# Algolzw/image-restoration-sde

Hardware: AMD Instinct MI355X
Metric: restored images/sec at 256x256, 100-step IR-SDE reverse sampler (higher is better)
Workload: dtype f32; 1 GPU; IR-SDE deraining ConditionalUNet nf=64 depth=4, reverse_sde, batch=16/GPU 256x256, T=100 (BASELINE.json configs[1]); compute_dtype=fp32, global_batch=16

## Files before the change

### image_restoration_sde_amd/csrc/common.h

```cpp
#pragma once
#include <hip/hip_runtime.h>
#include <cstdint>
#include <cstdio>
#include <cstdlib>
#include <stdexcept>
#include <string>
#include <vector>
#include "split3_layout.h"

namespace irsde {

struct HipError : std::runtime_error {
    using std::runtime_error::runtime_error;
};
struct HipOutOfMemory : HipError {
    using HipError::HipError;
};

inline int tuning_env_int(const char* name, int dflt) {
    static const bool on = [] { const char* t = getenv("IRSDE_TUNING"); return t && atoi(t) == 1; }();
    if (!on) return dflt;
    const char* v = getenv(name);
    return v ? atoi(v) : dflt;
}
// ... 77 lines not shown
struct WinoPolyParams {
    int up = 0;
    const float* in = nullptr;
    int C = 0, Hin = 0, Win = 0;
    int B = 0, TH = 0, TW = 0, T = 0;
    float* V = nullptr;
    unsigned short* Vs = nullptr;
    int thread_writer = 0;
    const float* M = nullptr;
    int Cout = 0, Ho = 0, Wo = 0;
    float* out = nullptr;
    int out_stride = 0;
    const float* bias = nullptr;
};
void launch_wino_poly_input(const WinoPolyParams& p, hipStream_t s);
void launch_wino_poly_output(const WinoPolyParams& p, hipStream_t s);
void wino_poly_transform_weights(const float* w_packed, int Cout, int Cin, float* U, int up);
struct SplitGemmArgs {
    const unsigned short* a = nullptr;
    const unsigned short* b = nullptr;
    float* out = nullptr;
    long long plA = 0, plB = 0, pA = 0, pB = 0, pO = 0;
    int M = 0, N = 0, K = 0, lda = 0, ldc = 0;
    float out_scale = 1.f;
    int n_inner = 1;
    int nblk_n = 0;
};
void gemm_split_global_init();
int gemm_split_inner(int M, int N, int ncomp);
void launch_gemm_split_pairs(const SplitGemmArgs& a, int ncomp, hipStream_t s, int abl = 0, bool f16 = false);
void launch_split_pairs(const float* in, unsigned short* out, size_t rows, int K, hipStream_t s, bool f16 = false,
                        float scale = 1.0f);
void launch_gemm_split(const SplitGemmArgs& a, int nplanes, int ncomp, hipStream_t s);
void launch_gemm_split_triples(const SplitGemmArgs& a, int ncomp, hipStream_t s, int abl = 0, int walk = -1);
void set_force_split3_blocks(int n);
bool gemm_split_triples_fits(long long M, long long N, long long K, long long ldc);
void launch_split_triples(const float* in, unsigned short* out, int ncomp, size_t rows, int K, hipStream_t s);
void launch_split_planes(const float* in, unsigned short* out, size_t n, size_t plane, int nplanes, hipStream_t s, bool f16 = false,
                         float scale = 1.0f);
void launch_wino_output(const WinoParams& p, hipStream_t s);
void wino_transform_weights(const float* w_packed, int Cout, int Cin, float* U, int tile);
bool wino_fused_eligible(const ConvParams& p);
void wino_fused_pack_weights(const float* U, int Cout, int Cin, float* Uf);
void launch_wino_fused(const ConvParams& p, const float* Uf, hipStream_t s, unsigned long long* dbg = nullptr, int dflags = 0);
int wino_fused_num_blocks(const ConvParams& p);
bool wino_fused64_eligible(const ConvParams& p);
void wino_fused64_pack_weights(const float* U, int Cout, int Cin, float* Uf);
void launch_wino_fused64(const ConvParams& p, const float* Uf, hipStream_t s, int variant = 0);
void wino_fused64_set_debug(unsigned long long* buf);
constexpr float kWinoFused64PairVScale = 0.0625f;
void launch_wino_fused64_split_weights(const float* Uf, unsigned short* out, size_t nfloats, float scale, hipStream_t s);
int wino_fused64_num_blocks(const ConvParams& p);
bool wino_fused64_xcd_nb(const ConvParams& p);
void wino_fused_global_init();
int device_cu_count();
bool wino_fused64t_eligible(const ConvParams& p);
long long wino_fused64t_num_items(const ConvParams& p);
void launch_wino_fused64t(const ConvParams& p, const float* Uf, hipStream_t s, int variant = 0);
void wino_fused64t_set_debug(unsigned long long* buf);
void wino_fused_t_global_init();
void naf_chain_global_init();
void naf_chain_set_debug(unsigned long long* buf);
bool naf_chain_shape_ok(int H, int W, int c);
size_t naf_chain_weight_halves(int nblocks);
size_t naf_chain_vec_floats(int nblocks);
void launch_naf_chain(const float* x, float* out, const unsigned short* w, const float* vecs, int nblocks, int B, const float* film, int film_bstride,
                      int film_off, const float* cam, int cam_bstride, int cam_off, hipStream_t s, int variant = 0);
// ... 156 lines not shown
```

### image_restoration_sde_amd/csrc/engine_debug.hip

```cpp
#include "engine.h"
#include "../../include/irsde_hip_debug.h"

using namespace irsde;

namespace irsde {
namespace {

struct Scratch {
    hipStream_t s;
    std::vector<void*> bufs;
    explicit Scratch(hipStream_t s_) : s(s_) {}
    ~Scratch() {
        (void)hipStreamSynchronize(s);
        for (void* p : bufs) (void)hipFree(p);
    }
    Scratch(const Scratch&) = delete;
    Scratch& operator=(const Scratch&) = delete;
    template <class T> T* alloc(size_t n) {
        void* p = nullptr;
        IRSDE_HIP_CHECK(hipMalloc(&p, n * sizeof(T)));
        bufs.push_back(p);
        return static_cast<T*>(p);
    }
    float* upload(const float* host, size_t n) {
// ... 20 lines not shown
        if (e0) (void)hipEventDestroy(e0);
        if (e1) (void)hipEventDestroy(e1);
    }
    EventPair(const EventPair&) = delete;
    EventPair& operator=(const EventPair&) = delete;
};
template <class Run>
double time_launches(hipStream_t s, int iters, Run&& run) {
    EventPair ev;
    IRSDE_HIP_CHECK(hipEventRecord(ev.e0, s));
    for (int i = 0; i < iters; ++i) run();
    IRSDE_HIP_CHECK(hipEventRecord(ev.e1, s));
    IRSDE_HIP_CHECK(hipStreamSynchronize(s));
    float ms = 0.f;
    IRSDE_HIP_CHECK(hipEventElapsedTime(&ms, ev.e0, ev.e1));
    return ms / iters;
}

struct VariantScope {
    explicit VariantScope(int v) { conv_set_variant(v); }
    ~VariantScope() { conv_set_variant(0); }
};

bool code_in(const std::initializer_list<int>& codes, int c) { return std::find(codes.begin(), codes.end(), c) != codes.end(); }
bool debug_conv_code_known(int c) {
    return code_in({0, 1, 2, 3, 4, 5, 12, 13, 22, 23, 24, 25, 26, 27, 28, 48, 33, 34, 35, 36, 37, 42, 43, 44, 45, 46, 47, 55, 56, 62, 63, 204, 260, 261, 262, 263}, c) ||
           code_in({100, 103, 105, 106, 107, 150, 160, 161, 162, 163, 165, 166, 167, 170, 171, 172, 173}, c);
}
bool bench_conv_variant_known(int v) {
    return code_in({0, 3, 5, 6, 7, 50, 60, 61, 62, 63, 64, 65, 66, 67, 70, 71, 72, 73}, v) ||
           code_in({80, 81, 82, 412, 413, 421, 422, 423, 430, 431, 432, 434, 435, 460, 461, 462, 465, 467, 468, 469, 480, 481, 482}, v) ||
           code_in({2001, 2002, 2004, 4650, 4651, 4652, 4653}, v) ||
           (v >= 83 && v <= 82 + 255) ||
           (v >= 490 && v <= 499) ||
           (v >= 472 && v <= 476);
}

struct ScamHookArgs {
    const float* x;
    float* out;
    const float *norm_l_g, *norm_r_g, *l_proj1_w, *l_proj1_b, *r_proj1_w, *r_proj1_b, *l_proj2_w, *l_proj2_b, *r_proj2_w, *r_proj2_b, *beta, *gamma;
};
struct ScamHookDev {
    float *gl, *gr, *beta, *gamma;
    float *in2, *qv, *F;
    size_t vsz;
};
template <class ShapeCheck, class Prologue, class Tail>
void scam_hook(const ScamHookArgs& a, int B, int Hs, int Ws, int C, void* stream, ShapeCheck check_shape, Prologue prologue, Tail tail) {
    if (!a.x || !a.out || !a.norm_l_g || !a.norm_r_g || !a.l_proj1_w || !a.l_proj1_b || !a.r_proj1_w || !a.r_proj1_b || !a.l_proj2_w || !a.l_proj2_b ||
        !a.r_proj2_w || !a.r_proj2_b || !a.beta || !a.gamma)
        throw HipError("null argument");
    check_shape();
    hipStream_t s = reinterpret_cast<hipStream_t>(stream);
    conv_global_init();
    std::vector<float> wl, bl, wr, br;
    scam_pack_proj(a.l_proj1_w, a.l_proj1_b, a.l_proj2_w, a.l_proj2_b, C, wl, bl);
    scam_pack_proj(a.r_proj1_w, a.r_proj1_b, a.r_proj2_w, a.r_proj2_b, C, wr, br);
    Scratch mem(s);
    auto up = [&](const float* h, size_t n) {
        float* d = mem.alloc<float>(std::max<size_t>(n, 16));
        if (h) IRSDE_HIP_CHECK(hipMemcpy(d, h, n * 4, hipMemcpyHostToDevice));
        return d;
    };
    ScamHookDev d;
    d.gl = up(a.norm_l_g, C); d.gr = up(a.norm_r_g, C); d.beta = up(a.beta, C); d.gamma = up(a.gamma, C);
    float *dwl = up(wl.data(), wl.size()), *dbl = up(bl.data(), bl.size()), *dwr = up(wr.data(), wr.size()), *dbr = up(br.data(), br.size());
// ... 434 lines not shown
            if (f16) {
                unsigned short* dbf = mem.alloc<unsigned short>(pk.size());
                launch_f32_to_f16(dw, dbf, pk.size(), s);
                p.w_bf = dbf;
                p.f16 = 1;
            }
            const size_t npix_in = (size_t)B * Hin * Win, nout = (size_t)B * p.Ho * p.Wo * Cout;
            if (act) {
                auto to_bf = [&](const float* src, size_t n) {
                    unsigned short* d = mem.alloc<unsigned short>(n + 32);
                    launch_f32_to_bf16(src, d, n, s);
                    return reinterpret_cast<const float*>(d);
                };
                p.in0 = to_bf(in0, npix_in * C0);
                if (in1) p.in1 = to_bf(in1, npix_in * C1);
                if (res) p.res = to_bf(res, nout);
                ao = mem.alloc<unsigned short>(nout + 32);
                p.out = reinterpret_cast<float*>(ao);
                p.in_bf16 = p.out_bf16 = 1;
            }
            {
                const int halo_v = (naive == 162 || naive == 262 || naive == 166) ? 64 : (naive == 163 || naive == 263 || naive == 167) ? 65 : 0;
                VariantScope vs(halo_v ? halo_v : f16 ? (naive == 165 ? 61 : 0) : act ? (naive == 204 ? 0 : naive - 200) : (naive >= 100 ? naive - 100 : 0));
                launch_conv(p, s);
            }
            if (act) launch_bf16_to_f32(ao, out, nout, s);
        }
        IRSDE_HIP_CHECK(hipStreamSynchronize(s));
    });
}

int irsde_debug_split_gemm(const float* A, const float* Bm, float* C, int M, int N, int K, int ncomp, int nplanes, void* stream) {
    return guard([&] {
        if (nplanes != 2 && nplanes != 3 && (nplanes < 42 || nplanes > 45)) throw HipError("debug_split_gemm: nplanes must be 2, 3, 42, 43, 44 or 45");
        hipStream_t s = reinterpret_cast<hipStream_t>(stream);
        conv_global_init();
        const size_t na = (size_t)ncomp * M * K, nb = (size_t)ncomp * N * K;
        Scratch mem(s);
        if (nplanes == 43 || nplanes == 45) {
            if (!gemm_split_triples_fits(M, N, K, N)) throw HipError("debug_split_gemm: shape not eligible for the three-piece GEMM");
            const size_t ea = split3_comp_elems((size_t)M, (size_t)K), eb = split3_comp_elems((size_t)N, (size_t)K);
            unsigned short *ta = mem.alloc<unsigned short>(ea * ncomp), *tb = mem.alloc<unsigned short>(eb * ncomp);
            launch_split_triples(A, ta, ncomp, (size_t)M, K, s);
            launch_split_triples(Bm, tb, ncomp, (size_t)N, K, s);
            SplitGemmArgs gt;
            gt.a = ta; gt.b = tb; gt.out = C;
            gt.pA = (long long)ea; gt.pB = (long long)eb; gt.pO = (long long)M * N;
            gt.M = M; gt.N = N; gt.K = K; gt.lda = K; gt.ldc = N;
            launch_gemm_split_triples(gt, ncomp, s, 0, nplanes == 45 ? 0 : -1);
            IRSDE_HIP_CHECK(hipStreamSynchronize(s));
            return;
        }
        if (nplanes == 42 || nplanes == 44) {
            const bool f16 = nplanes == 44;
            const float sa = f16 ? 1.0f / 16.0f : 1.f, sb = f16 ? 64.0f : 1.f;
            unsigned short *pa = mem.alloc<unsigned short>(2 * na), *pb = mem.alloc<unsigned short>(2 * nb);
            launch_split_pairs(A, pa, (size_t)ncomp * M, K, s, f16, sa);
            launch_split_pairs(Bm, pb, (size_t)ncomp * N, K, s, f16, sb);
            SplitGemmArgs gp;
            gp.a = pa; gp.b = pb; gp.out = C;
            gp.pA = (long long)M * K; gp.pB = (long long)N * K; gp.pO = (long long)M * N;
            gp.M = M; gp.N = N; gp.K = K; gp.lda = K; gp.ldc = N;
            gp.out_scale = 1.0f / (sa * sb);
            launch_gemm_split_pairs(gp, ncomp, s, 0, f16);
            IRSDE_HIP_CHECK(hipStreamSynchronize(s));
            return;
        }
        unsigned short *da = mem.alloc<unsigned short>(na * nplanes), *db = mem.alloc<unsigned short>(nb * nplanes);
        launch_split_planes(A, da, na, na, nplanes, s);
        launch_split_planes(Bm, db, nb, nb, nplanes, s);
        SplitGemmArgs g;
        g.a = da; g.b = db; g.out = C;
        g.plA = (long long)na; g.plB = (long long)nb;
        g.pA = (long long)M * K; g.pB = (long long)N * K; g.pO = (long long)M * N;
        g.M = M; g.N = N; g.K = K; g.lda = K; g.ldc = N;
        g.n_inner = gemm_split_inner(M, N, ncomp);
        launch_gemm_split(g, nplanes, ncomp, s);
        IRSDE_HIP_CHECK(hipStreamSynchronize(s));
    });
}

int irsde_debug_force_chain_groups(int g) {
// ... 143 lines not shown
        float* dfilm = mem.alloc<float>((size_t)2 * Cout + 256);
        float* dz = dfilm + 2 * Cout;
        IRSDE_HIP_CHECK(hipMemset(dz, 0, 1024));
        p.zeros = dz;
        launch_fill_random(din, nin, 1, 1.0f, s);
        launch_fill_random(dw, nw, 2, 1.0f / sqrtf((float)(K * K * Cin)), s);
        launch_fill_random(dres, nout, 3, 1.0f, s);
        launch_fill_random(dfilm, (size_t)2 * Cout, 4, 0.3f, s);
        p.in0 = din; p.w = dw; p.out = dout; p.out_stride = Cout;
        const int halo_force = (variant == 64 || variant == 66) ? 64 : (variant == 65 || variant == 67) ? 65 : 0;
        if (halo_force) variant = variant <= 65 ? 62 : 63;
        if (variant >= 60 && variant <= 63) {
            unsigned short* dbf = mem.alloc<unsigned short>(nw);
            launch_f32_to_bf16(dw, dbf, nw, s);
            p.w_bf = dbf;
        }
        if (epi == 1) { p.film = dfilm; p.silu = 1; }
        if (epi == 2) { p.silu = 1; p.res = dres; p.res_stride = Cout; }
        if (variant == 63) {
            unsigned short* dabf = mem.alloc<unsigned short>(nin);
            launch_f32_to_bf16(din, dabf, nin, s);
            launch_f32_to_bf16(dout, reinterpret_cast<unsigned short*>(dres), nout / 2, s);
            p.in0 = reinterpret_cast<const float*>(dabf);
            p.in_bf16 = 1; p.out_bf16 = 1;
        }
        float* dU = nullptr;
        WinoPlan wp{};
        if (variant == 480 || variant == 481 || variant == 482) {
            unsigned short* dwp = mem.alloc<unsigned short>(2 * nw);
            launch_split_pairs(dw, dwp, (size_t)Cout, K * K * Cin, s, variant != 481, 64.0f);
            p.w_pair = dwp; p.pair_scale = 1.0f / 64.0f; p.f16 = variant != 481 ? 1 : 0;
            variant = variant == 482 ? 61 : 0;
        }
        if (variant >= 490 && variant <= 499) {
            if (K != 3 || stride != 1 || !wino_shape_ok(p, 4)) throw HipError("bench_conv: Winograd variants need an eligible 3x3 stride-1 layer");
            const long long T = (long long)B * (p.Ho / 4) * (p.Wo / 4);
            if (!gemm_split_triples_fits(T, Cout, Cin, Cout)) throw HipError("bench_conv: shape not eligible for the three-piece GEMM");
            const size_t ea = split3_comp_elems((size_t)T, (size_t)Cin), eb = split3_comp_elems((size_t)Cout, (size_t)Cin);
            float *vf = mem.alloc<float>((size_t)36 * T * Cin), *uf = mem.alloc<float>((size_t)36 * Cout * Cin), *mo = mem.alloc<float>((size_t)36 * T * Cout);
            unsigned short *vt = mem.alloc<unsigned short>(36 * ea), *ut = mem.alloc<unsigned short>(36 * eb);
            launch_fill_random(vf, (size_t)36 * T * Cin, 7, 1.0f, s);
            launch_fill_random(uf, (size_t)36 * Cout * Cin, 8, 0.05f, s);
            launch_split_triples(vf, vt, 36, (size_t)T, Cin, s);
            launch_split_triples(uf, ut, 36, (size_t)Cout, Cin, s);
            SplitGemmArgs gt;
            gt.a = vt; gt.b = ut; gt.out = mo;
            gt.pA = (long long)ea; gt.pB = (long long)eb; gt.pO = T * Cout;
            gt.M = (int)T; gt.N = Cout; gt.K = Cin; gt.lda = Cin; gt.ldc = Cout;
            const int walk = variant >= 495 ? 0 : -1, abl = variant - (variant >= 495 ? 495 : 490);
            for (int i = 0; i < 2; ++i) launch_gemm_split_triples(gt, 36, s, abl, walk);
            *ms_out = time_launches(s, iters, [&] { launch_gemm_split_triples(gt, 36, s, abl, walk); });
            return;
        }
        if (variant >= 472 && variant <= 476) {
            if (K != 3 || stride != 1 || !wino_shape_ok(p, 4)) throw HipError("bench_conv: Winograd variants need an eligible 3x3 stride-1 layer");
            const long long T = (long long)B * (p.Ho / 4) * (p.Wo / 4);
            float *vf = mem.alloc<float>((size_t)36 * T * Cin), *uf = mem.alloc<float>((size_t)36 * Cout * Cin), *mo = mem.alloc<float>((size_t)36 * T * Cout);
            unsigned short *vp = mem.alloc<unsigned short>((size_t)36 * T * Cin * 2), *up = mem.alloc<unsigned short>((size_t)36 * Cout * Cin * 2);
            launch_fill_random(vf, (size_t)36 * T * Cin, 7, 1.0f, s);
            launch_fill_random(uf, (size_t)36 * Cout * Cin, 8, 0.05f, s);
            launch_split_pairs(vf, vp, (size_t)36 * T, Cin, s);
            launch_split_pairs(uf, up, (size_t)36 * Cout, Cin, s);
            SplitGemmArgs gp;
            gp.a = vp; gp.b = up; gp.out = mo;
            gp.pA = T * Cin; gp.pB = (long long)Cout * Cin; gp.pO = T * Cout;
            gp.M = (int)T; gp.N = Cout; gp.K = Cin; gp.lda = Cin; gp.ldc = Cout;
            const int abl = variant - 472;
            for (int i = 0; i < 2; ++i) launch_gemm_split_pairs(gp, 36, s, abl);
            *ms_out = time_launches(s, iters, [&] { launch_gemm_split_pairs(gp, 36, s, abl); });
            return;
        }
        const bool split_v = variant == 412 || variant == 413 || variant == 422 || variant == 423;
        WinoSplitPlan sp{};
        if (variant == 80 || variant == 81 || variant == 421 || split_v || (variant >= 83 && variant <= 82 + 255) || (variant >= 430 && variant <= 469) || variant >= 2000) {
            if (K != 3 || stride != 1) throw HipError("bench_conv: Winograd variants need a 3x3 stride-1 layer");
            dU = mem.alloc<float>((size_t)36 * nw / 9);
            launch_fill_random(dU, (size_t)36 * nw / 9, 5, 1.0f / sqrtf((float)(9 * Cin)), s);
            if (variant != 81 && variant != 421 && !split_v && !wino_fused_eligible(p)) throw HipError("bench_conv: shape not eligible for the fused Winograd kernel");
            if (variant >= 400 && !wino_fused64_eligible(p)) throw HipError("bench_conv: shape not eligible for the 64-cout fused Winograd kernel");
            if (variant == 434) {
                float* dUp = mem.alloc<float>((size_t)36 * nw / 9);
                launch_wino_fused64_split_weights(dU, reinterpret_cast<unsigned short*>(dUp), (size_t)36 * nw / 9, 256.0f, s);
                dU = dUp;
                p.pair_scale = 1.0f / (kWinoFused64PairVScale * 256.0f);
// ... 153 lines not shown
```

### image_restoration_sde_amd/csrc/gemm_split.hip

```cpp
#include "common.h"
#include <algorithm>
#include <atomic>
#include <type_traits>

namespace irsde {

typedef float floatx16 __attribute__((ext_vector_type(16)));
typedef __bf16 bf16x8 __attribute__((ext_vector_type(8)));
typedef _Float16 f16x8 __attribute__((ext_vector_type(8)));
typedef unsigned uintx4 __attribute__((ext_vector_type(4)));

namespace {

constexpr int SG_BK = 32;
constexpr int SG_ROWB = 80;
constexpr int SG_PLANE = 128 * SG_ROWB;

template <int NPL>
__global__ __launch_bounds__(256, 1) void gemm_split_kernel(const SplitGemmArgs g) {
    constexpr int NPROD = NPL == 3 ? 6 : 3;
    constexpr int PA[6] = {0, 1, 2, 0, 1, 0};
    constexpr int PB[6] = {2, 1, 0, 1, 0, 0};
    constexpr int P0 = 6 - NPROD;
    constexpr int A_BYTES = NPL * SG_PLANE;
// ... 264 lines not shown
        const char* a = lds + buf * STAGE + wm * TM * 32 * 128;
        const char* b = lds + buf * STAGE + A_STAGE + wn * TN * 32 * 128;
        frag_t fa[2][2][TM], fb[2][2][TN];
#pragma unroll
        for (int sb = 0; sb < 2; ++sb)
#pragma unroll
            for (int p = 0; p < 2; ++p) {
#pragma unroll
                for (int i = 0; i < TM; ++i) fa[sb][p][i] = *reinterpret_cast<const frag_t*>(a + i * 32 * 128 + fr_off[p][sb]);
#pragma unroll
                for (int j = 0; j < TN; ++j) fb[sb][p][j] = *reinterpret_cast<const frag_t*>(b + j * 32 * 128 + fr_off[p][sb]);
            }
        __builtin_amdgcn_sched_barrier(0);
#pragma unroll
        for (int sb = 0; sb < 2; ++sb)
#pragma unroll
            for (int pr = 0; pr < 3; ++pr) {
#pragma unroll
                for (int i = 0; i < TM; ++i)
#pragma unroll
                    for (int j = 0; j < TN; ++j)
                        if (ABL != 3) {
                            if constexpr (F16) acc[i][j] = __builtin_amdgcn_mfma_f32_32x32x16_f16(fa[sb][pr == 1 ? 1 : 0][i], fb[sb][pr == 0 ? 1 : 0][j], acc[i][j], 0, 0, 0);
                            else acc[i][j] = __builtin_amdgcn_mfma_f32_32x32x16_bf16(fa[sb][pr == 1 ? 1 : 0][i], fb[sb][pr == 0 ? 1 : 0][j], acc[i][j], 0, 0, 0);
                        }
                        else acc[i][j][0] += (float)fa[sb][pr == 1 ? 1 : 0][i][0] * (float)fb[sb][pr == 0 ? 1 : 0][j][0];
                if (sb == 0 && ABL != 1 && more) issue_loads_part(buf ^ 1, pr);
                __builtin_amdgcn_sched_barrier(0);
            }
        __syncthreads();
    }
    flush(0);
}
template <int ABL = 0, bool WALK = true>
__global__ __launch_bounds__(512, 1) void gemm_split3i_kernel(const SplitGemmArgs g) {
    constexpr int TM = 2, TN = 2, WN = 2, BM = 256, BN = 128;
    constexpr int ROWB = 192, GROUP = 16 * ROWB;
    constexpr int A_STAGE = BM * ROWB, STAGE = (BM + BN) * ROWB;
    constexpr int PA[6] = {0, 1, 2, 0, 1, 0};
    constexpr int PB[6] = {2, 1, 0, 1, 0, 0};
    extern __shared__ __attribute__((aligned(16))) char lds[];
    const int tid = threadIdx.x, lane = tid & 63;
    const int wave = __builtin_amdgcn_readfirstlane(tid >> 6);
    const int wm = wave / WN, wn = wave % WN;
    const int l31 = lane & 31, h = lane >> 5;
    const int mtiles = (g.M + BM - 1) / BM;
    const int units = mtiles * g.n_inner;
    const int xcd = blockIdx.x & 7, jx = blockIdx.x >> 3;
    const int ulo = (int)((long long)xcd * units / 8), uhi = (int)((long long)(xcd + 1) * units / 8);
    const int nitems = (uhi - ulo) * g.nblk_n;
    const int it_step = WALK ? ((int)gridDim.x - xcd + 7) >> 3 : nitems;
    int it = jx;
    if (it >= nitems) return;
    const int nk = g.K / SG_BK;
    const unsigned pairb = (unsigned)nk * 384u;

    int plane0, m0, n0;
    unsigned a_voff[6], b_voff[3];
    const char *acomp, *bcomp;
    auto set_item = [&](int i) {
        const int unit = ulo + i / g.nblk_n, nblk = i % g.nblk_n;
        plane0 = unit / mtiles;
        m0 = (unit - plane0 * mtiles) * BM;
        n0 = nblk * BN;
#pragma unroll
        for (int q = 0; q < 9; ++q) {
            const int gi = q / 3, wl = q - gi * 3;
            const int sl = wl * 64 + lane;
            const int r = sl / 12, pos = sl - r * 12;
            int j = pos - ((r >> 2) & 3);
            j = j < 0 ? j + 12 : j;
            if (gi < 2) {
                int m = m0 + (2 * wave + gi) * 16 + r;
                m = m < g.M ? m : g.M - 1;
                a_voff[q] = (unsigned)(m >> 1) * pairb + (unsigned)(m & 1) * 192u + (unsigned)j * 16u;
            } else {
                int n = n0 + wave * 16 + r;
                n = n < g.N ? n : g.N - 1;
                b_voff[wl] = (unsigned)(n >> 1) * pairb + (unsigned)(n & 1) * 192u + (unsigned)j * 16u;
            }
        }
        acomp = reinterpret_cast<const char*>(g.a) + (long long)plane0 * g.pA * 2;
        bcomp = reinterpret_cast<const char*>(g.b) + (long long)plane0 * g.pB * 2;
    };
    int kb = 0;
    auto issue_loads_part = [&](int buf, int part) {
        const char* gsrc = (part < 2 ? acomp : bcomp) + (size_t)kb * 384;
        char* l = lds + buf * STAGE + (part < 2 ? (2 * wave + part) * GROUP : A_STAGE + wave * GROUP);
#pragma unroll
        for (int wl = 0; wl < 3; ++wl) IRSDE_GLDS16(gsrc + (part < 2 ? a_voff[part * 3 + wl] : b_voff[wl]), l + wl * 1024);
    };

    floatx16 acc[TM][TN];
#pragma unroll
    for (int i = 0; i < TM; ++i)
#pragma unroll
        for (int j = 0; j < TN; ++j)
#pragma unroll
            for (int r = 0; r < 16; ++r) acc[i][j][r] = 0.f;

    set_item(it);
#pragma unroll
    for (int part = 0; part < 3; ++part) issue_loads_part(0, part);

    int fr_off[3][2];
#pragma unroll
    for (int p = 0; p < 3; ++p)
#pragma unroll
        for (int sb = 0; sb < 2; ++sb) fr_off[p][sb] = l31 * ROWB + ((p * 4 + sb * 2 + h + ((l31 >> 2) & 3)) % 12) * 16;
    for (;;) {
        __syncthreads();
        for (int st = 0; st < nk; ++st) {
            const int buf = st & 1;
            const bool more = st + 1 < nk;
            if (more) ++kb;
            const char* a = lds + buf * STAGE + wm * TM * 32 * ROWB;
            const char* b = lds + buf * STAGE + A_STAGE + wn * TN * 32 * ROWB;
            bf16x8 fa[2][3][TM], fb[2][3][TN];
#pragma unroll
            for (int sb = 0; sb < 2; ++sb)
#pragma unroll
                for (int p = 0; p < 3; ++p) {
#pragma unroll
                    for (int i = 0; i < TM; ++i) fa[sb][p][i] = *reinterpret_cast<const bf16x8*>(a + i * 32 * ROWB + fr_off[p][sb]);
#pragma unroll
                    for (int j = 0; j < TN; ++j) fb[sb][p][j] = *reinterpret_cast<const bf16x8*>(b + j * 32 * ROWB + fr_off[p][sb]);
                }
            __builtin_amdgcn_sched_barrier(0);
#pragma unroll
            for (int sb = 0; sb < 2; ++sb)
#pragma unroll
                for (int pr = 0; pr < 6; ++pr) {
#pragma unroll
                    for (int i = 0; i < TM; ++i)
#pragma unroll
                        for (int j = 0; j < TN; ++j) {
                            if (ABL != 3) acc[i][j] = __builtin_amdgcn_mfma_f32_32x32x16_bf16(fa[sb][PA[pr]][i], fb[sb][PB[pr]][j], acc[i][j], 0, 0, 0);
                            else acc[i][j][0] += (float)fa[sb][PA[pr]][i][0] * (float)fb[sb][PB[pr]][j][0];
                        }
                    if (sb == 0 && pr < 3 && ABL != 1 && more) issue_loads_part(buf ^ 1, pr);
                    __builtin_amdgcn_sched_barrier(0);
                }
            __syncthreads();
        }

        const int rowb_ = m0 + wm * TM * 32, colb = n0 + wn * TN * 32;
        float* ob = g.out + (long long)plane0 * g.pO + (long long)rowb_ * g.ldc;
        const int rows = g.M - rowb_;
        const unsigned nrec = rows <= 0 ? 0u : (unsigned)(rows < TM * 32 ? rows : TM * 32) * (unsigned)g.ldc * 4u;
        const __amdgpu_buffer_rsrc_t ro = __builtin_amdgcn_make_buffer_rsrc(ob, 0, nrec, 0x00020000);
        it += it_step;
        const bool next = WALK && it < nitems;
        if (next) {
            set_item(it);
            kb = 0;
#pragma unroll
            for (int part = 0; part < 3; ++part) issue_loads_part(0, part);
            __builtin_amdgcn_sched_barrier(0);
        }
#pragma unroll
        for (int i = 0; i < TM; ++i)
#pragma unroll
            for (int j = 0; j < TN; ++j) {
                const int colu = colb + j * 32;
                if (colu + l31 < g.N && (ABL != 4 || acc[i][j][0] == 1.2345e30f)) {
#pragma unroll
                    for (int r = 0; r < 16; ++r) {
                        const float v = acc[i][j][r];
                        const unsigned voff = (unsigned)((i * 32 + (r & 3) + 8 * (r >> 2) + 4 * h) * g.ldc + colu + l31) * 4u;
                        __builtin_amdgcn_raw_buffer_store_b32(__builtin_bit_cast(unsigned, v), ro, (int)voff, 0, 0);
                    }
                }
            }
        if (!next) break;
#pragma unroll
        for (int i = 0; i < TM; ++i)
#pragma unroll
            for (int j = 0; j < TN; ++j)
#pragma unroll
                for (int r = 0; r < 16; ++r) acc[i][j][r] = 0.f;
    }
}
#undef IRSDE_GLDS16

__global__ __launch_bounds__(256) void split_triples_kernel(const float* __restrict__ in, unsigned short* __restrict__ out, const size_t n, const size_t rows,
                                                            const int K) {
    const size_t i = (size_t)blockIdx.x * blockDim.x + threadIdx.x;
    if (i >= n) return;
    const size_t rk = rows * (size_t)K;
    const size_t z = i / rk, rem = i - z * rk;
    const size_t row = rem / K;
    const int k = (int)(rem - row * K);
    float r = in[i];
    unsigned short* o = out + z * split3_comp_elems(rows, K);
#pragma unroll
    for (int p = 0; p < 3; ++p) {
        const __bf16 hb = (__bf16)r;
        o[split3_index(row, k, p, K / 32)] = __builtin_bit_cast(unsigned short, hb);
        r -= (float)hb;
    }
}

template <bool F16>
__global__ __launch_bounds__(256) void split_pairs_kernel(const float* __restrict__ in, unsigned short* __restrict__ out, const size_t n, const int K,
                                                          const float scale) {
    const size_t i = (size_t)blockIdx.x * blockDim.x + threadIdx.x;
    if (i >= n) return;
    const size_t row = i / K;
    const int k = (int)(i - row * K);
    float r = in[i];
    const size_t base = (row * (size_t)(K / 32) + k / 32) * 64 + (k & 31);
    if constexpr (F16) {
        r *= scale;
        const _Float16 hb = (_Float16)r;
        out[base] = __builtin_bit_cast(unsigned short, hb);
// ... 10 lines not shown
}

template <int NPL, bool F16 = false>
__global__ __launch_bounds__(256) void split_planes_kernel(const float* __restrict__ in, unsigned short* __restrict__ out, const size_t n,
                                                           const size_t plane, const float scale) {
    const size_t i = (size_t)blockIdx.x * blockDim.x + threadIdx.x;
    if (i >= n) return;
    float r = F16 ? in[i] * scale : in[i];
#pragma unroll
    for (int p = 0; p < NPL; ++p) {
        if constexpr (F16) {
            const _Float16 hb = (_Float16)r;
            out[p * plane + i] = __builtin_bit_cast(unsigned short, hb);
            r -= (float)hb;
        } else {
            const __bf16 hb = (__bf16)r;
            out[p * plane + i] = __builtin_bit_cast(unsigned short, hb);
            r -= (float)hb;
        }
    }
}

}

void gemm_split_global_init() {
    IRSDE_HIP_CHECK(hipFuncSetAttribute(reinterpret_cast<const void*>(gemm_split2i_kernel<0>), hipFuncAttributeMaxDynamicSharedMemorySize, 160 * 1024));
    IRSDE_HIP_CHECK(hipFuncSetAttribute(reinterpret_cast<const void*>(gemm_split2i_kernel<0, true>), hipFuncAttributeMaxDynamicSharedMemorySize, 160 * 1024));
    IRSDE_HIP_CHECK(hipFuncSetAttribute(reinterpret_cast<const void*>(gemm_split2i_kernel<5, true>), hipFuncAttributeMaxDynamicSharedMemorySize, 160 * 1024));
    IRSDE_HIP_CHECK(hipFuncSetAttribute(reinterpret_cast<const void*>(gemm_split2i_kernel<1>), hipFuncAttributeMaxDynamicSharedMemorySize, 160 * 1024));
    IRSDE_HIP_CHECK(hipFuncSetAttribute(reinterpret_cast<const void*>(gemm_split2i_kernel<3>), hipFuncAttributeMaxDynamicSharedMemorySize, 160 * 1024));
    IRSDE_HIP_CHECK(hipFuncSetAttribute(reinterpret_cast<const void*>(gemm_split2i_kernel<4>), hipFuncAttributeMaxDynamicSharedMemorySize, 160 * 1024));
    IRSDE_HIP_CHECK(hipFuncSetAttribute(reinterpret_cast<const void*>(gemm_split3i_kernel<0, true>), hipFuncAttributeMaxDynamicSharedMemorySize, 160 * 1024));
    IRSDE_HIP_CHECK(hipFuncSetAttribute(reinterpret_cast<const void*>(gemm_split3i_kernel<0, false>), hipFuncAttributeMaxDynamicSharedMemorySize, 160 * 1024));
#ifdef IRSDE_PROBES
    IRSDE_HIP_CHECK(hipFuncSetAttribute(reinterpret_cast<const void*>(gemm_split3i_kernel<1, true>), hipFuncAttributeMaxDynamicSharedMemorySize, 160 * 1024));
    IRSDE_HIP_CHECK(hipFuncSetAttribute(reinterpret_cast<const void*>(gemm_split3i_kernel<3, true>), hipFuncAttributeMaxDynamicSharedMemorySize, 160 * 1024));
    IRSDE_HIP_CHECK(hipFuncSetAttribute(reinterpret_cast<const void*>(gemm_split3i_kernel<4, true>), hipFuncAttributeMaxDynamicSharedMemorySize, 160 * 1024));
    IRSDE_HIP_CHECK(hipFuncSetAttribute(reinterpret_cast<const void*>(gemm_split3i_kernel<1, false>), hipFuncAttributeMaxDynamicSharedMemorySize, 160 * 1024));
    IRSDE_HIP_CHECK(hipFuncSetAttribute(reinterpret_cast<const void*>(gemm_split3i_kernel<3, false>), hipFuncAttributeMaxDynamicSharedMemorySize, 160 * 1024));
    IRSDE_HIP_CHECK(hipFuncSetAttribute(reinterpret_cast<const void*>(gemm_split3i_kernel<4, false>), hipFuncAttributeMaxDynamicSharedMemorySize, 160 * 1024));
#endif
    IRSDE_HIP_CHECK(hipFuncSetAttribute(reinterpret_cast<const void*>(gemm_split_kernel<2>), hipFuncAttributeMaxDynamicSharedMemorySize, 160 * 1024));
    IRSDE_HIP_CHECK(hipFuncSetAttribute(reinterpret_cast<const void*>(gemm_split_kernel<3>), hipFuncAttributeMaxDynamicSharedMemorySize, 160 * 1024));
}

int gemm_split_inner(int M, int N, int ncomp) {
    const long long tiles = (long long)((M + 127) / 128) * ((N + 127) / 128);
    for (int d = ncomp; d >= 1; --d)
        if (ncomp % d == 0 && tiles * (ncomp / d) >= 512) return d;
    return 1;
}

void launch_gemm_split_pairs(const SplitGemmArgs& a, int ncomp, hipStream_t s, int abl, bool f16) {
    if (a.K % SG_BK) throw HipError("gemm_split_pairs: K must be a multiple of 32");
    if ((unsigned long long)a.M * a.K * 4ull >= 0xffffffffull || (unsigned long long)a.N * a.K * 4ull >= 0xffffffffull ||
        (size_t)a.M * a.ldc * 4 >= 0xffffffffull)
        throw HipError("gemm_split_pairs: a component exceeds the 32-bit offset range");
    SplitGemmArgs g = a;
    g.nblk_n = (a.N + 255) / 256;
    g.n_inner = ncomp;
    const int units = ((a.M + 255) / 256) * ncomp;
    int per_xcd = 0;
    for (int x = 0; x < 8; ++x) per_xcd = std::max(per_xcd, (int)((long long)(x + 1) * units / 8) - (int)((long long)x * units / 8));
    const dim3 grid((unsigned)(8 * per_xcd * g.nblk_n));
    const size_t lds = (size_t)2 * 512 * 128;
    if (f16) {
        if (abl != 0) throw HipError("gemm_split_pairs: the ablation twins exist for the bf16 kernel only");
        static const bool nt = tuning_env_int("IRSDE_SPLIT_NT", 0) != 0;
        if (nt) hipLaunchKernelGGL((gemm_split2i_kernel<5, true>), grid, dim3(512), lds, s, g);
        else hipLaunchKernelGGL((gemm_split2i_kernel<0, true>), grid, dim3(512), lds, s, g);
        IRSDE_HIP_CHECK(hipGetLastError());
        return;
    }
    switch (abl) {
        case 0: hipLaunchKernelGGL(gemm_split2i_kernel<0>, grid, dim3(512), lds, s, g); break;
        case 1: hipLaunchKernelGGL(gemm_split2i_kernel<1>, grid, dim3(512), lds, s, g); break;
        case 3: hipLaunchKernelGGL(gemm_split2i_kernel<3>, grid, dim3(512), lds, s, g); break;
        case 4: hipLaunchKernelGGL(gemm_split2i_kernel<4>, grid, dim3(512), lds, s, g); break;
        default: throw HipError("gemm_split_pairs: bad ablation variant");
    }
    IRSDE_HIP_CHECK(hipGetLastError());
}

bool gemm_split_triples_fits(long long M, long long N, long long K, long long ldc) {
    if (M < 1 || N < 1 || K < 32 || K % SG_BK) return false;
    return (unsigned long long)split3_comp_elems((size_t)M, (size_t)K) * 2ull < 0xffffffffull && (unsigned long long)split3_comp_elems((size_t)N, (size_t)K) * 2ull < 0xffffffffull &&
           (unsigned long long)M * ldc * 4ull < 0xffffffffull;
}

static std::atomic<int> g_force_split3_blocks{-1};
void set_force_split3_blocks(int n) { g_force_split3_blocks.store(n >= 8 ? n : -1, std::memory_order_relaxed); }

void launch_gemm_split_triples(const SplitGemmArgs& a, int ncomp, hipStream_t s, int abl, int walk) {
    if (a.K % SG_BK) throw HipError("gemm_split_triples: K must be a multiple of 32");
    if (!gemm_split_triples_fits(a.M, a.N, a.K, a.ldc)) throw HipError("gemm_split_triples: a component exceeds the 32-bit offset range");
    if (ncomp < 1 || a.ldc < a.N) throw HipError("gemm_split_triples: bad component count or output stride");
    if (walk < 0) {
        static const int knob = tuning_env_int("IRSDE_SPLIT3_WALK", 1);
        walk = knob != 0;
    }
    SplitGemmArgs g = a;
    g.nblk_n = (a.N + 127) / 128;
    g.n_inner = ncomp;
    const long long units = (long long)((a.M + 255) / 256) * ncomp;
    long long per_xcd = 0;
    for (int x = 0; x < 8; ++x) per_xcd = std::max(per_xcd, (x + 1) * units / 8 - x * units / 8);
    long long blocks = 8 * per_xcd * g.nblk_n;
    if (blocks >= 0x7fffffffll) throw HipError("gemm_split_triples: grid too large");
    if (walk) {
        const int forced = g_force_split3_blocks.load(std::memory_order_relaxed);
        blocks = std::min<long long>(blocks, std::max(8, forced > 0 ? forced : device_cu_count()));
    }
    const dim3 grid((unsigned)blocks);
    const size_t lds = (size_t)2 * (256 + 128) * 192;
    switch (abl * 2 + (walk ? 1 : 0)) {
        case 1: hipLaunchKernelGGL((gemm_split3i_kernel<0, true>), grid, dim3(512), lds, s, g); break;
        case 0: hipLaunchKernelGGL((gemm_split3i_kernel<0, false>), grid, dim3(512), lds, s, g); break;
#ifdef IRSDE_PROBES
        case 3: hipLaunchKernelGGL((gemm_split3i_kernel<1, true>), grid, dim3(512), lds, s, g); break;
        case 7: hipLaunchKernelGGL((gemm_split3i_kernel<3, true>), grid, dim3(512), lds, s, g); break;
        case 9: hipLaunchKernelGGL((gemm_split3i_kernel<4, true>), grid, dim3(512), lds, s, g); break;
        case 2: hipLaunchKernelGGL((gemm_split3i_kernel<1, false>), grid, dim3(512), lds, s, g); break;
        case 6: hipLaunchKernelGGL((gemm_split3i_kernel<3, false>), grid, dim3(512), lds, s, g); break;
        case 8: hipLaunchKernelGGL((gemm_split3i_kernel<4, false>), grid, dim3(512), lds, s, g); break;
#endif
        default: throw HipError("gemm_split_triples: the ablation twins are part of the PROBES build");
    }
    IRSDE_HIP_CHECK(hipGetLastError());
}

void launch_split_triples(const float* in, unsigned short* out, int ncomp, size_t rows, int K, hipStream_t s) {
    if (K % 32 || ncomp < 1 || rows < 1) throw HipError("split_triples: K must be a multiple of 32");
    const size_t n = (size_t)ncomp * rows * (size_t)K;
    hipLaunchKernelGGL(split_triples_kernel, dim3((unsigned)((n + 255) / 256)), dim3(256), 0, s, in, out, n, rows, K);
    IRSDE_HIP_CHECK(hipGetLastError());
}

void launch_split_pairs(const float* in, unsigned short* out, size_t rows, int K, hipStream_t s, bool f16, float scale) {
    if (K % 32) throw HipError("split_pairs: K must be a multiple of 32");
    const size_t n = rows * (size_t)K;
    if (f16) hipLaunchKernelGGL(split_pairs_kernel<true>, dim3((unsigned)((n + 255) / 256)), dim3(256), 0, s, in, out, n, K, scale);
    else hipLaunchKernelGGL(split_pairs_kernel<false>, dim3((unsigned)((n + 255) / 256)), dim3(256), 0, s, in, out, n, K, 1.0f);
    IRSDE_HIP_CHECK(hipGetLastError());
}

void launch_gemm_split(const SplitGemmArgs& a, int nplanes, int ncomp, hipStream_t s) {
    if (nplanes != 2 && nplanes != 3) throw HipError("gemm_split: 2 or 3 planes");
    if (a.K % SG_BK || a.n_inner < 1 || ncomp % a.n_inner) throw HipError("gemm_split: K must be a multiple of 32, n_inner a divisor of the component count");
    if ((size_t)a.M * a.ldc * 4 >= 0xffffffffull) throw HipError("gemm_split: output plane exceeds the 32-bit buffer range");
    SplitGemmArgs g = a;
    g.nblk_n = (a.N + 127) / 128;
    const dim3 grid((unsigned)(((a.M + 127) / 128) * g.nblk_n), (unsigned)(ncomp / a.n_inner));
    const size_t lds = (size_t)4 * nplanes * SG_PLANE;
    if (nplanes == 3) hipLaunchKernelGGL(gemm_split_kernel<3>, grid, dim3(256), lds, s, g);
    else hipLaunchKernelGGL(gemm_split_kernel<2>, grid, dim3(256), lds, s, g);
    IRSDE_HIP_CHECK(hipGetLastError());
}
// ... 13 lines not shown
```

Measured before the change: 4.730 images/s.

## Deepen split3 GEMM pipeline with interleaved fragment reads and split barriers

Restructures the three-piece bf16 GEMM main loop so LDS fragment reads for the next sub-step and the next stage overlap MFMA work, and global-to-LDS loads are issued two stages ahead, spread across waves (early/late halves). Full __syncthreads are replaced by vmcnt waits plus an LDS-only barrier, with a mid-stage barrier per M sub-tile. The A-row wave mapping changes to match. Also adds a DRAIN twin (env knob, default off) for probing. This lowers register use for A fragments and aims to hide load latency, at the cost of more barriers and tighter ordering assumptions about double-buffer reuse.

Result: faster. 4.809 images/s (median of 6 runs) (+1.7%).

```diff
diff --git a/image_restoration_sde_amd/csrc/common.h b/image_restoration_sde_amd/csrc/common.h
--- a/image_restoration_sde_amd/csrc/common.h
+++ b/image_restoration_sde_amd/csrc/common.h
@@ -133,7 +133,7 @@
 void launch_split_pairs(const float* in, unsigned short* out, size_t rows, int K, hipStream_t s, bool f16 = false,
                         float scale = 1.0f);
 void launch_gemm_split(const SplitGemmArgs& a, int nplanes, int ncomp, hipStream_t s);
-void launch_gemm_split_triples(const SplitGemmArgs& a, int ncomp, hipStream_t s, int abl = 0, int walk = -1);
+void launch_gemm_split_triples(const SplitGemmArgs& a, int ncomp, hipStream_t s, int abl = 0, int walk = -1, int drain = -1);
 void set_force_split3_blocks(int n);
 bool gemm_split_triples_fits(long long M, long long N, long long K, long long ldc);
 void launch_split_triples(const float* in, unsigned short* out, int ncomp, size_t rows, int K, hipStream_t s);
diff --git a/image_restoration_sde_amd/csrc/engine_debug.hip b/image_restoration_sde_amd/csrc/engine_debug.hip
--- a/image_restoration_sde_amd/csrc/engine_debug.hip
+++ b/image_restoration_sde_amd/csrc/engine_debug.hip
@@ -76,7 +76,7 @@
            code_in({80, 81, 82, 412, 413, 421, 422, 423, 430, 431, 432, 434, 435, 460, 461, 462, 465, 467, 468, 469, 480, 481, 482}, v) ||
            code_in({2001, 2002, 2004, 4650, 4651, 4652, 4653}, v) ||
            (v >= 83 && v <= 82 + 255) ||
-           (v >= 490 && v <= 499) ||
+           (v >= 490 && v <= 504) ||
            (v >= 472 && v <= 476);
 }
 
@@ -577,12 +577,12 @@
 
 int irsde_debug_split_gemm(const float* A, const float* Bm, float* C, int M, int N, int K, int ncomp, int nplanes, void* stream) {
     return guard([&] {
-        if (nplanes != 2 && nplanes != 3 && (nplanes < 42 || nplanes > 45)) throw HipError("debug_split_gemm: nplanes must be 2, 3, 42, 43, 44 or 45");
+        if (nplanes != 2 && nplanes != 3 && (nplanes < 42 || nplanes > 45) && nplanes != 47) throw HipError("debug_split_gemm: nplanes must be 2, 3, 42, 43, 44, 45 or 47");
         hipStream_t s = reinterpret_cast<hipStream_t>(stream);
         conv_global_init();
         const size_t na = (size_t)ncomp * M * K, nb = (size_t)ncomp * N * K;
         Scratch mem(s);
-        if (nplanes == 43 || nplanes == 45) {
+        if (nplanes == 43 || nplanes == 45 || nplanes == 47) {
             if (!gemm_split_triples_fits(M, N, K, N)) throw HipError("debug_split_gemm: shape not eligible for the three-piece GEMM");
             const size_t ea = split3_comp_elems((size_t)M, (size_t)K), eb = split3_comp_elems((size_t)N, (size_t)K);
             unsigned short *ta = mem.alloc<unsigned short>(ea * ncomp), *tb = mem.alloc<unsigned short>(eb * ncomp);
@@ -592,7 +592,7 @@
             gt.a = ta; gt.b = tb; gt.out = C;
             gt.pA = (long long)ea; gt.pB = (long long)eb; gt.pO = (long long)M * N;
             gt.M = M; gt.N = N; gt.K = K; gt.lda = K; gt.ldc = N;
-            launch_gemm_split_triples(gt, ncomp, s, 0, nplanes == 45 ? 0 : -1);
+            launch_gemm_split_triples(gt, ncomp, s, 0, nplanes == 45 ? 0 : nplanes == 47 ? 1 : -1, nplanes == 47 ? 1 : nplanes == 43 ? -1 : 0);
             IRSDE_HIP_CHECK(hipStreamSynchronize(s));
             return;
         }
@@ -802,7 +802,7 @@
             p.w_pair = dwp; p.pair_scale = 1.0f / 64.0f; p.f16 = variant != 481 ? 1 : 0;
             variant = variant == 482 ? 61 : 0;
         }
-        if (variant >= 490 && variant <= 499) {
+        if (variant >= 490 && variant <= 504) {
             if (K != 3 || stride != 1 || !wino_shape_ok(p, 4)) throw HipError("bench_conv: Winograd variants need an eligible 3x3 stride-1 layer");
             const long long T = (long long)B * (p.Ho / 4) * (p.Wo / 4);
             if (!gemm_split_triples_fits(T, Cout, Cin, Cout)) throw HipError("bench_conv: shape not eligible for the three-piece GEMM");
@@ -817,9 +817,10 @@
             gt.a = vt; gt.b = ut; gt.out = mo;
             gt.pA = (long long)ea; gt.pB = (long long)eb; gt.pO = T * Cout;
             gt.M = (int)T; gt.N = Cout; gt.K = Cin; gt.lda = Cin; gt.ldc = Cout;
-            const int walk = variant >= 495 ? 0 : -1, abl = variant - (variant >= 495 ? 495 : 490);
-            for (int i = 0; i < 2; ++i) launch_gemm_split_triples(gt, 36, s, abl, walk);
-            *ms_out = time_launches(s, iters, [&] { launch_gemm_split_triples(gt, 36, s, abl, walk); });
+            const int twin = (variant - 490) / 5, abl = (variant - 490) % 5;
+            const int walk = twin == 1 ? 0 : twin == 2 ? 1 : -1, drain = twin == 2 ? 1 : twin == 1 ? 0 : -1;
+            for (int i = 0; i < 2; ++i) launch_gemm_split_triples(gt, 36, s, abl, walk, drain);
+            *ms_out = time_launches(s, iters, [&] { launch_gemm_split_triples(gt, 36, s, abl, walk, drain); });
             return;
         }
         if (variant >= 472 && variant <= 476) {
diff --git a/image_restoration_sde_amd/csrc/gemm_split.hip b/image_restoration_sde_amd/csrc/gemm_split.hip
--- a/image_restoration_sde_amd/csrc/gemm_split.hip
+++ b/image_restoration_sde_amd/csrc/gemm_split.hip
@@ -320,7 +320,13 @@
     }
     flush(0);
 }
-template <int ABL = 0, bool WALK = true>
+#define IRSDE_WAIT_VM(N) asm volatile("s_waitcnt vmcnt(" #N ")" ::: "memory")
+#define IRSDE_PHASE_BARRIER()                              \
+    do {                                                   \
+        asm volatile("s_waitcnt lgkmcnt(0)" ::: "memory"); \
+        __builtin_amdgcn_s_barrier();                      \
+    } while (0)
+template <int ABL = 0, bool WALK = true, bool DRAIN = false>
 __global__ __launch_bounds__(512, 1) void gemm_split3i_kernel(const SplitGemmArgs g) {
     constexpr int TM = 2, TN = 2, WN = 2, BM = 256, BN = 128;
     constexpr int ROWB = 192, GROUP = 16 * ROWB;
@@ -343,6 +349,7 @@
     const int nk = g.K / SG_BK;
     const unsigned pairb = (unsigned)nk * 384u;
 
+    const int ga0 = 4 * (wave >> 1) + (wave & 1);
     int plane0, m0, n0;
     unsigned a_voff[6], b_voff[3];
     const char *acomp, *bcomp;
@@ -359,7 +366,7 @@
             int j = pos - ((r >> 2) & 3);
             j = j < 0 ? j + 12 : j;
             if (gi < 2) {
-                int m = m0 + (2 * wave + gi) * 16 + r;
+                int m = m0 + (ga0 + 2 * gi) * 16 + r;
                 m = m < g.M ? m : g.M - 1;
                 a_voff[q] = (unsigned)(m >> 1) * pairb + (unsigned)(m & 1) * 192u + (unsigned)j * 16u;
             } else {
@@ -371,12 +378,25 @@
         acomp = reinterpret_cast<const char*>(g.a) + (long long)plane0 * g.pA * 2;
         bcomp = reinterpret_cast<const char*>(g.b) + (long long)plane0 * g.pB * 2;
     };
-    int kb = 0;
-    auto issue_loads_part = [&](int buf, int part) {
-        const char* gsrc = (part < 2 ? acomp : bcomp) + (size_t)kb * 384;
-        char* l = lds + buf * STAGE + (part < 2 ? (2 * wave + part) * GROUP : A_STAGE + wave * GROUP);
-#pragma unroll
-        for (int wl = 0; wl < 3; ++wl) IRSDE_GLDS16(gsrc + (part < 2 ? a_voff[part * 3 + wl] : b_voff[wl]), l + wl * 1024);
+    auto issue_unit = [&](int kb, int kind) {
+        const char* gsrc = (kind < 2 ? acomp : bcomp) + (size_t)kb * 384;
+        char* l = lds + (kb & 1) * STAGE + (kind < 2 ? (ga0 + 2 * kind) * GROUP : A_STAGE + wave * GROUP);
+#pragma unroll
+        for (int wl = 0; wl < 3; ++wl) IRSDE_GLDS16(gsrc + (kind < 2 ? a_voff[kind * 3 + wl] : b_voff[wl]), l + wl * 1024);
+    };
+    auto issue_one = [&](int kb, int kind, int wl) {
+        const char* gsrc = (kind < 2 ? acomp : bcomp) + (size_t)kb * 384;
+        char* l = lds + (kb & 1) * STAGE + (kind < 2 ? (ga0 + 2 * kind) * GROUP : A_STAGE + wave * GROUP);
+        IRSDE_GLDS16(gsrc + (kind < 2 ? a_voff[kind * 3 + wl] : b_voff[wl]), l + wl * 1024);
+    };
+    auto issue_first = [&]() {
+        issue_unit(0, 0);
+        issue_unit(0, 2);
+        issue_unit(0, 1);
+        if (nk > 1) {
+            issue_unit(1, 0);
+            issue_unit(1, 2);
+        }
     };
 
     floatx16 acc[TM][TN];
@@ -388,48 +408,76 @@
             for (int r = 0; r < 16; ++r) acc[i][j][r] = 0.f;
 
     set_item(it);
-#pragma unroll
-    for (int part = 0; part < 3; ++part) issue_loads_part(0, part);
+    issue_first();
 
     int fr_off[3][2];
 #pragma unroll
     for (int p = 0; p < 3; ++p)
 #pragma unroll
         for (int sb = 0; sb < 2; ++sb) fr_off[p][sb] = l31 * ROWB + ((p * 4 + sb * 2 + h + ((l31 >> 2) & 3)) % 12) * 16;
+    bf16x8 fa[2][3], fb[2][3][TN];
+    auto read_a = [&](int sb, const char* a) {
+#pragma unroll
+        for (int p = 0; p < 3; ++p) fa[sb][p] = *reinterpret_cast<const bf16x8*>(a + fr_off[p][sb]);
+    };
+    auto read_b = [&](int sb, const char* b) {
+#pragma unroll
+        for (int p = 0; p < 3; ++p)
+#pragma unroll
+            for (int j = 0; j < TN; ++j) fb[sb][p][j] = *reinterpret_cast<const bf16x8*>(b + j * 32 * ROWB + fr_off[p][sb]);
+    };
+    const bool late = wave >= 4;
+    const int a_base = wm * TM * 32 * ROWB, b_base = A_STAGE + wn * TN * 32 * ROWB;
     for (;;) {
-        __syncthreads();
+        IRSDE_WAIT_VM(0);
+        IRSDE_PHASE_BARRIER();
+        read_a(0, lds + a_base);
+        read_b(0, lds + b_base);
+        __builtin_amdgcn_sched_barrier(0);
         for (int st = 0; st < nk; ++st) {
-            const int buf = st & 1;
-            const bool more = st + 1 < nk;
-            if (more) ++kb;
-            const char* a = lds + buf * STAGE + wm * TM * 32 * ROWB;
-            const char* b = lds + buf * STAGE + A_STAGE + wn * TN * 32 * ROWB;
-            bf16x8 fa[2][3][TM], fb[2][3][TN];
-#pragma unroll
-            for (int sb = 0; sb < 2; ++sb)
-#pragma unroll
-                for (int p = 0; p < 3; ++p) {
-#pragma unroll
-                    for (int i = 0; i < TM; ++i) fa[sb][p][i] = *reinterpret_cast<const bf16x8*>(a + i * 32 * ROWB + fr_off[p][sb]);
-#pragma unroll
-                    for (int j = 0; j < TN; ++j) fb[sb][p][j] = *reinterpret_cast<const bf16x8*>(b + j * 32 * ROWB + fr_off[p][sb]);
-                }
-            __builtin_amdgcn_sched_barrier(0);
-#pragma unroll
-            for (int sb = 0; sb < 2; ++sb)
-#pragma unroll
-                for (int pr = 0; pr < 6; ++pr) {
-#pragma unroll
-                    for (int i = 0; i < TM; ++i)
-#pragma unroll
-                        for (int j = 0; j < TN; ++j) {
-                            if (ABL != 3) acc[i][j] = __builtin_amdgcn_mfma_f32_32x32x16_bf16(fa[sb][PA[pr]][i], fb[sb][PB[pr]][j], acc[i][j], 0, 0, 0);
-                            else acc[i][j][0] += (float)fa[sb][PA[pr]][i][0] * (float)fb[sb][PB[pr]][j][0];
-                        }
-                    if (sb == 0 && pr < 3 && ABL != 1 && more) issue_loads_part(buf ^ 1, pr);
+            const bool more1 = st + 1 < nk, more2 = st + 2 < nk;
+            const char* a = lds + (st & 1) * STAGE + a_base;
+            const char* b = lds + (st & 1) * STAGE + b_base;
+            const char* an = lds + ((st + 1) & 1) * STAGE + a_base;
+            const char* bn = lds + ((st + 1) & 1) * STAGE + b_base;
+#pragma unroll
+            for (int i = 0; i < TM; ++i) {
+                if (i == 1) {
+                    read_a(0, a + 32 * ROWB);
                     __builtin_amdgcn_sched_barrier(0);
                 }
-            __syncthreads();
+#pragma unroll
+                for (int sb = 0; sb < 2; ++sb)
+#pragma unroll
+                    for (int pr = 0; pr < 6; ++pr) {
+#pragma unroll
+                        for (int j = 0; j < TN; ++j) {
+                            if (ABL != 3) acc[i][j] = __builtin_amdgcn_mfma_f32_32x32x16_bf16(fa[sb][PA[pr]], fb[sb][PB[pr]][j], acc[i][j], 0, 0, 0);
+                            else acc[i][j][0] += (float)fa[sb][PA[pr]][0] * (float)fb[sb][PB[pr]][j][0];
+                        }
+                        __builtin_amdgcn_sched_barrier(0);
+                        if (sb == 0 && pr == 0) {
+                            if (i == 0) {
+                                read_a(1, a);
+                                read_b(1, b);
+                            } else {
+                                read_a(1, a + 32 * ROWB);
+                            }
+                        }
+                        if (i == 1 && sb == 1 && pr == 0 && more1) {
+                            read_a(0, an);
+                            read_b(0, bn);
+                        }
+                        if (ABL != 1 && (sb == 1) == late) {
+                            if (i == 0 && pr >= 1 && pr <= 3 && more1) issue_one(st + 1, 1, pr - 1);
+                            if (i == 1 && more2) issue_one(st + 2, pr < 3 ? 0 : 2, pr % 3);
+                        }
+                        __builtin_amdgcn_sched_barrier(0);
+                    }
+                if (DRAIN || (i == 0 && !more1)) IRSDE_WAIT_VM(0);
+                else if (i == 0) IRSDE_WAIT_VM(3);
+                IRSDE_PHASE_BARRIER();
+            }
         }
 
         const int rowb_ = m0 + wm * TM * 32, colb = n0 + wn * TN * 32;
@@ -441,9 +489,7 @@
         const bool next = WALK && it < nitems;
         if (next) {
             set_item(it);
-            kb = 0;
-#pragma unroll
-            for (int part = 0; part < 3; ++part) issue_loads_part(0, part);
+            issue_first();
             __builtin_amdgcn_sched_barrier(0);
         }
 #pragma unroll
@@ -469,6 +515,8 @@
                 for (int r = 0; r < 16; ++r) acc[i][j][r] = 0.f;
     }
 }
+#undef IRSDE_PHASE_BARRIER
+#undef IRSDE_WAIT_VM
 #undef IRSDE_GLDS16
 
 __global__ __launch_bounds__(256) void split_triples_kernel(const float* __restrict__ in, unsigned short* __restrict__ out, const size_t n, const size_t rows,
@@ -545,6 +593,7 @@
     IRSDE_HIP_CHECK(hipFuncSetAttribute(reinterpret_cast<const void*>(gemm_split2i_kernel<4>), hipFuncAttributeMaxDynamicSharedMemorySize, 160 * 1024));
     IRSDE_HIP_CHECK(hipFuncSetAttribute(reinterpret_cast<const void*>(gemm_split3i_kernel<0, true>), hipFuncAttributeMaxDynamicSharedMemorySize, 160 * 1024));
     IRSDE_HIP_CHECK(hipFuncSetAttribute(reinterpret_cast<const void*>(gemm_split3i_kernel<0, false>), hipFuncAttributeMaxDynamicSharedMemorySize, 160 * 1024));
+    IRSDE_HIP_CHECK(hipFuncSetAttribute(reinterpret_cast<const void*>(gemm_split3i_kernel<0, true, true>), hipFuncAttributeMaxDynamicSharedMemorySize, 160 * 1024));
 #ifdef IRSDE_PROBES
     IRSDE_HIP_CHECK(hipFuncSetAttribute(reinterpret_cast<const void*>(gemm_split3i_kernel<1, true>), hipFuncAttributeMaxDynamicSharedMemorySize, 160 * 1024));
     IRSDE_HIP_CHECK(hipFuncSetAttribute(reinterpret_cast<const void*>(gemm_split3i_kernel<3, true>), hipFuncAttributeMaxDynamicSharedMemorySize, 160 * 1024));
@@ -552,6 +601,9 @@
     IRSDE_HIP_CHECK(hipFuncSetAttribute(reinterpret_cast<const void*>(gemm_split3i_kernel<1, false>), hipFuncAttributeMaxDynamicSharedMemorySize, 160 * 1024));
     IRSDE_HIP_CHECK(hipFuncSetAttribute(reinterpret_cast<const void*>(gemm_split3i_kernel<3, false>), hipFuncAttributeMaxDynamicSharedMemorySize, 160 * 1024));
     IRSDE_HIP_CHECK(hipFuncSetAttribute(reinterpret_cast<const void*>(gemm_split3i_kernel<4, false>), hipFuncAttributeMaxDynamicSharedMemorySize, 160 * 1024));
+    IRSDE_HIP_CHECK(hipFuncSetAttribute(reinterpret_cast<const void*>(gemm_split3i_kernel<1, true, true>), hipFuncAttributeMaxDynamicSharedMemorySize, 160 * 1024));
+    IRSDE_HIP_CHECK(hipFuncSetAttribute(reinterpret_cast<const void*>(gemm_split3i_kernel<3, true, true>), hipFuncAttributeMaxDynamicSharedMemorySize, 160 * 1024));
+    IRSDE_HIP_CHECK(hipFuncSetAttribute(reinterpret_cast<const void*>(gemm_split3i_kernel<4, true, true>), hipFuncAttributeMaxDynamicSharedMemorySize, 160 * 1024));
 #endif
     IRSDE_HIP_CHECK(hipFuncSetAttribute(reinterpret_cast<const void*>(gemm_split_kernel<2>), hipFuncAttributeMaxDynamicSharedMemorySize, 160 * 1024));
     IRSDE_HIP_CHECK(hipFuncSetAttribute(reinterpret_cast<const void*>(gemm_split_kernel<3>), hipFuncAttributeMaxDynamicSharedMemorySize, 160 * 1024));
@@ -604,7 +656,7 @@
 static std::atomic<int> g_force_split3_blocks{-1};
 void set_force_split3_blocks(int n) { g_force_split3_blocks.store(n >= 8 ? n : -1, std::memory_order_relaxed); }
 
-void launch_gemm_split_triples(const SplitGemmArgs& a, int ncomp, hipStream_t s, int abl, int walk) {
+void launch_gemm_split_triples(const SplitGemmArgs& a, int ncomp, hipStream_t s, int abl, int walk, int drain) {
     if (a.K % SG_BK) throw HipError("gemm_split_triples: K must be a multiple of 32");
     if (!gemm_split_triples_fits(a.M, a.N, a.K, a.ldc)) throw HipError("gemm_split_triples: a component exceeds the 32-bit offset range");
     if (ncomp < 1 || a.ldc < a.N) throw HipError("gemm_split_triples: bad component count or output stride");
@@ -612,6 +664,11 @@
         static const int knob = tuning_env_int("IRSDE_SPLIT3_WALK", 1);
         walk = knob != 0;
     }
+    if (drain < 0) {
+        static const int knob = tuning_env_int("IRSDE_SPLIT3_DRAIN", 0);
+        drain = knob != 0;
+    }
+    if (drain && !walk) throw HipError("gemm_split_triples: the drain twin exists on the walk only");
     SplitGemmArgs g = a;
     g.nblk_n = (a.N + 127) / 128;
     g.n_inner = ncomp;
@@ -626,9 +683,10 @@
     }
     const dim3 grid((unsigned)blocks);
     const size_t lds = (size_t)2 * (256 + 128) * 192;
-    switch (abl * 2 + (walk ? 1 : 0)) {
+    switch (abl * 2 + (walk ? 1 : 0) + (drain ? 100 : 0)) {
         case 1: hipLaunchKernelGGL((gemm_split3i_kernel<0, true>), grid, dim3(512), lds, s, g); break;
         case 0: hipLaunchKernelGGL((gemm_split3i_kernel<0, false>), grid, dim3(512), lds, s, g); break;
+        case 101: hipLaunchKernelGGL((gemm_split3i_kernel<0, true, true>), grid, dim3(512), lds, s, g); break;
 #ifdef IRSDE_PROBES
         case 3: hipLaunchKernelGGL((gemm_split3i_kernel<1, true>), grid, dim3(512), lds, s, g); break;
         case 7: hipLaunchKernelGGL((gemm_split3i_kernel<3, true>), grid, dim3(512), lds, s, g); break;
@@ -636,6 +694,9 @@
         case 2: hipLaunchKernelGGL((gemm_split3i_kernel<1, false>), grid, dim3(512), lds, s, g); break;
         case 6: hipLaunchKernelGGL((gemm_split3i_kernel<3, false>), grid, dim3(512), lds, s, g); break;
         case 8: hipLaunchKernelGGL((gemm_split3i_kernel<4, false>), grid, dim3(512), lds, s, g); break;
+        case 103: hipLaunchKernelGGL((gemm_split3i_kernel<1, true, true>), grid, dim3(512), lds, s, g); break;
+        case 107: hipLaunchKernelGGL((gemm_split3i_kernel<3, true, true>), grid, dim3(512), lds, s, g); break;
+        case 109: hipLaunchKernelGGL((gemm_split3i_kernel<4, true, true>), grid, dim3(512), lds, s, g); break;
 #endif
         default: throw HipError("gemm_split_triples: the ablation twins are part of the PROBES build");
     }
```
